# ReactiveBayes/RxInfer.jl

Hardware: NVIDIA H100
Metric: gaussian_messages_per_sec_batched_lgssm_d4_T1000 (higher is better)
Workload: dtype f32

## Files before the change

rxinfer.jl_b200/csrc/rxg_gain.cuh:

```cuda
#pragma once
#include <cooperative_groups.h>

#include "rxg_lgssm_common.cuh"

namespace rxg {
namespace cg = cooperative_groups;

constexpr int GS_CTAS = 8;
constexpr int GS_THREADS = 128;
constexpr int GS_NT = GS_CTAS * GS_THREADS;

struct ScanWs {
    double* fel;
    double* ftot;
    double* bel;
    double* btot;
};

template <int R, int C>
__device__ __forceinline__ Mat<double, R, C> ldcg_d(const double* p) {
    Mat<double, R, C> o;
#pragma unroll
    for (int i = 0; i < R * C; ++i) o.a[i] = __ldcg(p + i);
    return o;
}
template <int R, int C>
__device__ __forceinline__ Mat<double, R, C> ld_soa_d(const double* p, size_t n, size_t i) {
    Mat<double, R, C> o;
#pragma unroll
    for (int c = 0; c < R * C; ++c) o.a[c] = __ldcg(p + (size_t)c * n + i);
    return o;
}
template <int R, int C>
__device__ __forceinline__ void st_soa_d(double* p, size_t n, size_t i, const Mat<double, R, C>& A) {
#pragma unroll
    for (int c = 0; c < R * C; ++c) p[(size_t)c * n + i] = A.a[c];
}

template <int N, int K>
__device__ __forceinline__ Mat<double, N, K> solve_general(Mat<double, N, N> Mx, Mat<double, N, K> Rh) {
#pragma unroll
    for (int c = 0; c < N; ++c) {
        int p = c;
        double best = fabs(Mx(c, c));
#pragma unroll
        for (int r = c + 1; r < N; ++r) {
            const double v = fabs(Mx(r, c));
            if (v > best) { best = v; p = r; }
        }
#pragma unroll
        for (int r = c + 1; r < N; ++r) {
            if (r == p) {
#pragma unroll
                for (int j = c; j < N; ++j) { const double t = Mx(c, j); Mx(c, j) = Mx(r, j); Mx(r, j) = t; }
#pragma unroll
                for (int j = 0; j < K; ++j) { const double t = Rh(c, j); Rh(c, j) = Rh(r, j); Rh(r, j) = t; }
            }
        }
        const double inv = 1.0 / Mx(c, c);
#pragma unroll
        for (int r = c + 1; r < N; ++r) {
            const double f = Mx(r, c) * inv;
#pragma unroll
            for (int j = c + 1; j < N; ++j) Mx(r, j) = fma(-f, Mx(c, j), Mx(r, j));
#pragma unroll
            for (int j = 0; j < K; ++j) Rh(r, j) = fma(-f, Rh(c, j), Rh(r, j));
        }
    }
    Mat<double, N, K> X;
#pragma unroll
// ... 46 lines not shown
    Mat<double, D, D> Mx = mul(ei.C, ej.J);
#pragma unroll
    for (int i = 0; i < D; ++i) Mx(i, i) += 1.0;
    Mat<double, D, 2 * D> Rh;
#pragma unroll
    for (int i = 0; i < D; ++i)
#pragma unroll
        for (int j = 0; j < D; ++j) { Rh(i, j) = ei.A(i, j); Rh(i, D + j) = ei.C(i, j); }
    Mat<double, D, 2 * D> X = solve_general<D, 2 * D>(Mx, Rh);
    Mat<double, D, D> X1, X2;
#pragma unroll
    for (int i = 0; i < D; ++i)
#pragma unroll
        for (int j = 0; j < D; ++j) { X1(i, j) = X(i, j); X2(i, j) = X(i, D + j); }
    FwdEl<D> o;
    Mat<double, D, D> T2 = mul(ej.A, X2);
    o.C = sym_mul_nt_add(T2, ej.A, ej.C);
    if (!C_ONLY) {
        o.A = mul(ej.A, X1);
        Mat<double, D, D> JX = mul(ej.J, X1);
        Mat<double, D, D> AtJX = mul_tn(ei.A, JX);
#pragma unroll
        for (int i = 0; i < D; ++i)
#pragma unroll
            for (int j = 0; j <= i; ++j) {
                const double s = 0.5 * (AtJX(i, j) + AtJX(j, i)) + ei.J(i, j);
                o.J(i, j) = s; o.J(j, i) = s;
            }
    }
    return o;
}

template <int D>
__device__ __forceinline__ void bwd_store(double* p, size_t n, size_t i, const BwdEl<D>& e) {
    st_soa_d<D, D>(p, n, i, e.E);
    st_soa_d<D, D>(p + (size_t)D * D * n, n, i, e.L);
}
template <int D>
__device__ __forceinline__ BwdEl<D> bwd_load(const double* p, size_t n, size_t i) {
    BwdEl<D> e;
    e.E = ld_soa_d<D, D>(p, n, i);
    e.L = ld_soa_d<D, D>(p + (size_t)D * D * n, n, i);
    return e;
}
template <int D, bool L_ONLY>
__device__ __forceinline__ BwdEl<D> bwd_combine(const BwdEl<D>& early, const BwdEl<D>& late) {
    BwdEl<D> o;
    Mat<double, D, D> EL = mul(early.E, late.L);
    o.L = sym_mul_nt_add(EL, early.E, early.L);
    if (!L_ONLY) o.E = mul(early.E, late.E);
    return o;
}

template <int D, int M>
__global__ void __cluster_dims__(GS_CTAS, 1, 1) __launch_bounds__(GS_THREADS, 1)
gain_scan_kernel(const __grid_constant__ ModelF<D, M> mdl, GainWs ws, ScanWs sw, int T, int transition_first,
                 float* __restrict__ cov_shared_out, int* __restrict__ bad_out, const uint8_t* __restrict__ tmask,
                 const float* __restrict__ useq) {
    using TB = Tab<D, M>;
    cg::cluster_group cluster = cg::this_cluster();
    const int g = (int)cluster.block_rank() * GS_THREADS + (int)threadIdx.x;
    const int E = (T + GS_NT - 1) / GS_NT;
    const int k0 = g * E, k1 = min(k0 + E, T);
    constexpr int FE = 3 * D * D, BE = 2 * D * D;
    bool bad = false;

    const Mat<double, D, D> A = load_const<double, D, D>(mdl.A), P = load_const<double, D, D>(mdl.P);
    const Mat<double, M, D> B = load_const<double, M, D>(mdl.B);
    const Mat<double, M, M> Q = load_const<double, M, M>(mdl.Q);

    {
        FwdEl<D> acc = fwd_identity<D>();
        if (k0 < k1) {
            FwdEl<D> gen;
            {
                Mat<double, M, D> BP = mul(B, P);
                Mat<double, M, M> Sinn = sym_mul_nt_add(BP, B, Q);
                Chol<double, M> ch = cholesky<double, M, false>(Sinn, bad);
                Mat<double, D, M> V = solve_right_Lt(transpose(BP), ch.L);
                Mat<double, D, M> K = solve_right_L(V, ch.L);
                Mat<double, D, D> IKB = identity<double, D>();
#pragma unroll
                for (int i = 0; i < D; ++i)
#pragma unroll
                    for (int j = 0; j < D; ++j)
#pragma unroll
                        for (int k = 0; k < M; ++k) IKB(i, j) -= K(i, k) * B(k, j);
                gen.A = mul(IKB, A);
                gen.C = sym_downdate(P, V);
                Mat<double, M, D> BA = mul(B, A);
                Mat<double, M, D> Wm;
#pragma unroll
                for (int c = 0; c < D; ++c) {
                    Vec<double, M> col;
#pragma unroll
                    for (int r = 0; r < M; ++r) col(r) = BA(r, c);
                    Vec<double, M> z = solve_L(ch.L, col);
#pragma unroll
                    for (int r = 0; r < M; ++r) Wm(r, c) = z(r);
                }
                Mat<double, D, D> Z;
#pragma unroll
                for (int i = 0; i < D * D; ++i) Z.a[i] = 0.0;
                gen.J = sym_mul_nt_add(transpose(Wm), transpose(Wm), Z);
            }
            for (int k = k0; k < k1; ++k) {
                if (k == 0) {
                    Mat<double, D, D> S = load_const<double, D, D>(mdl.S0);
                    if (transition_first) { Mat<double, D, D> AS = mul(A, S); S = sym_mul_nt_add(AS, A, P); }
                    FwdEl<D> first;
#pragma unroll
                    for (int i = 0; i < D * D; ++i) { first.A.a[i] = 0.0; first.J.a[i] = 0.0; }
                    if (!tmask || tmask[0] != 0) {
                        Mat<double, M, D> BS = mul(B, S);
                        Mat<double, M, M> Sinn = sym_mul_nt_add(BS, B, Q);
                        Chol<double, M> ch = cholesky<double, M, false>(Sinn, bad);
                        Mat<double, D, M> V = solve_right_Lt(transpose(BS), ch.L);
                        first.C = sym_downdate(S, V);
                    } else {
                        first.C = S;
                    }
                    acc = first;
                } else {
                    const bool obs_k = !tmask || tmask[k] != 0;
                    if (obs_k) {
                        acc = (k == k0) ? gen : fwd_combine<D, false>(acc, gen);
                    } else {
                        FwdEl<D> miss;
                        miss.A = A; miss.C = P;
#pragma unroll
                        for (int i = 0; i < D * D; ++i) miss.J.a[i] = 0.0;
                        acc = (k == k0) ? miss : fwd_combine<D, false>(acc, miss);
                    }
                }
                if (E > 1) fwd_store<D>(sw.fel, T, k, acc);
            }
        }
        fwd_store<D>(sw.ftot, GS_NT, g, acc);
    }
    cluster.sync();
    int cur = 0;
    for (int off = 1; off < GS_NT; off <<= 1) {
        const double* src = sw.ftot + (size_t)cur * GS_NT * FE;
        double* dst = sw.ftot + (size_t)(cur ^ 1) * GS_NT * FE;
        FwdEl<D> mine = fwd_load<D>(src, GS_NT, g);
        if (g >= off && (g - off) * E < T && k0 < T) {
            FwdEl<D> prev = fwd_load<D>(src, GS_NT, g - off);
            mine = fwd_combine<D, false>(prev, mine);
        }
        fwd_store<D>(dst, GS_NT, g, mine);
        cluster.sync();
        cur ^= 1;
    }
    {
        const double* tot = sw.ftot + (size_t)cur * GS_NT * FE;
        if (E == 1) {
            if (g < T) store_d(ws.Sf + (size_t)g * D * D, ld_soa_d<D, D>(tot + (size_t)D * D * GS_NT, GS_NT, g));
        } else if (k0 < k1) {
            if (g == 0) {
                for (int k = k0; k < k1; ++k)
                    store_d(ws.Sf + (size_t)k * D * D, ld_soa_d<D, D>(sw.fel + (size_t)D * D * T, T, k));
            } else {
                const FwdEl<D> excl = fwd_load<D>(tot, GS_NT, g - 1);
                for (int k = k0; k < k1; ++k) {
                    const FwdEl<D> pk = fwd_load<D>(sw.fel, T, k);
                    store_d(ws.Sf + (size_t)k * D * D, fwd_combine<D, true>(excl, pk).C);
                }
            }
        }
    }
    cluster.sync();
    for (int t = g; t < T; t += GS_NT) {
        const Mat<double, D, D> Sf = ldcg_d<D, D>(ws.Sf + (size_t)t * D * D);
        Mat<double, D, D> Sp;
        if (t > 0) {
            Mat<double, D, D> Sfm = ldcg_d<D, D>(ws.Sf + (size_t)(t - 1) * D * D);
            Mat<double, D, D> AS = mul(A, Sfm);
            Sp = sym_mul_nt_add(AS, A, P);
        } else {
            Sp = load_const<double, D, D>(mdl.S0);
            if (transition_first) { Mat<double, D, D> AS = mul(A, Sp); Sp = sym_mul_nt_add(AS, A, P); }
        }
        const bool obs_t = !tmask || tmask[t] != 0;
        {
            Mat<double, D, M> K;
            Mat<double, M, M> Li;
            double cconst = 0.0;
#pragma unroll
            for (int i = 0; i < D * M; ++i) K.a[i] = 0.0;
#pragma unroll
            for (int i = 0; i < M * M; ++i) Li.a[i] = 0.0;
            if (obs_t) {
                Mat<double, M, D> BS = mul(B, Sp);
                Mat<double, M, M> Sinn = sym_mul_nt_add(BS, B, Q);
                Chol<double, M> ch = cholesky<double, M, true>(Sinn, bad);
                Mat<double, D, M> V = solve_right_Lt(transpose(BS), ch.L);
                K = solve_right_L(V, ch.L);
#pragma unroll
                for (int j = 0; j < M; ++j) {
                    Li(j, j) = ch.L(j, j);
#pragma unroll
                    for (int i = j + 1; i < M; ++i) {
                        double sacc = 0.0;
#pragma unroll
                        for (int k = j; k < i; ++k) sacc -= ch.L(i, k) * Li(k, j);
                        Li(i, j) = sacc * ch.L(i, i);
                    }
                }
                cconst = M * RXG_HALF_LOG_2PI - ch.neg_half_logdet;
            }
            Mat<double, D, D> IKB = identity<double, D>();
#pragma unroll
            for (int i = 0; i < D; ++i)
#pragma unroll
                for (int j = 0; j < D; ++j)
#pragma unroll
                    for (int k = 0; k < M; ++k) IKB(i, j) -= K(i, k) * B(k, j);
            Mat<double, D, D> F = (t > 0 || transition_first) ? mul(IKB, A) : IKB;
            float* rec = ws.fwd + (size_t)t * TB::FWD_REC;
            store_f(rec + TB::F_OFF, F);
            store_f(rec + TB::K_OFF, K);
            store_f(rec + TB::LI_OFF, Li);
            rec[TB::C_OFF] = (float)cconst;
            Vec<double, D> uu, gf;
#pragma unroll
            for (int i = 0; i < D; ++i) uu(i) = (double)(useq ? useq[(size_t)t * D + i] : mdl.u[i]);
            gf = mulv(IKB, uu);
            if (!(t > 0 || transition_first)) {
#pragma unroll
                for (int i = 0; i < D; ++i) gf(i) = 0.0;
            }
            store_fv(rec + TB::GF_OFF, gf);
            store_f(ws.sf + (size_t)t * TB::SF_REC, Sf);
        }
        float* brec = ws.bwd + (size_t)t * TB::BWD_REC;
        BwdEl<D> be;
        Vec<double, D> gb;
#pragma unroll
        for (int i = 0; i < D; ++i) gb(i) = 0.0;
        if (t < T - 1) {
            Mat<double, D, D> AS = mul(A, Sf);
            Mat<double, D, D> Sp1 = sym_mul_nt_add(AS, A, P);
            Chol<double, D> ch = cholesky<double, D, false>(Sp1, bad);
            Mat<double, D, D> U = solve_right_Lt(transpose(AS), ch.L);
            be.E = solve_right_L(U, ch.L);
            be.L = sym_downdate(Sf, U);
            Mat<double, D, D> Em = identity<double, D>();
            Mat<double, D, D> GA = mul(be.E, A);
#pragma unroll
            for (int i = 0; i < D * D; ++i) Em.a[i] -= GA.a[i];
            store_f(brec + TB::E_OFF, Em);
            store_f(brec + TB::G_OFF, be.E);
            Vec<double, D> uu;
#pragma unroll
            for (int i = 0; i < D; ++i) uu(i) = -(double)(useq ? useq[(size_t)(t + 1) * D + i] : mdl.u[i]);
            gb = mulv(be.E, uu);
        } else {
#pragma unroll
            for (int i = 0; i < D * D; ++i) be.E.a[i] = 0.0;
            be.L = Sf;
            store_f(brec + TB::E_OFF, identity<double, D>());
            store_f(brec + TB::G_OFF, be.E);
        }
        store_fv(brec + TB::GB_OFF, gb);
        bwd_store<D>(sw.bel, T, t, be);
    }
    cluster.sync();
    {
        BwdEl<D> acc;
        acc.E = identity<double, D>();
#pragma unroll
        for (int i = 0; i < D * D; ++i) acc.L.a[i] = 0.0;
        for (int r = k0; r < k1; ++r) {
            const int t = T - 1 - r;
            const BwdEl<D> el = bwd_load<D>(sw.bel, T, t);
            acc = (r == k0) ? el : bwd_combine<D, false>(el, acc);
            if (E > 1) bwd_store<D>(sw.bel, T, t, acc);
        }
        bwd_store<D>(sw.btot, GS_NT, g, acc);
    }
    cluster.sync();
    cur = 0;
    for (int off = 1; off < GS_NT; off <<= 1) {
        const double* src = sw.btot + (size_t)cur * GS_NT * BE;
        double* dst = sw.btot + (size_t)(cur ^ 1) * GS_NT * BE;
        BwdEl<D> mine = bwd_load<D>(src, GS_NT, g);
        if (g >= off && k0 < T) {
            BwdEl<D> prev = bwd_load<D>(src, GS_NT, g - off);
            mine = bwd_combine<D, false>(mine, prev);
        }
        bwd_store<D>(dst, GS_NT, g, mine);
        cluster.sync();
        cur ^= 1;
    }
    {
        const double* tot = sw.btot + (size_t)cur * GS_NT * BE;
        BwdEl<D> excl;
        if (E > 1 && g > 0 && k0 < k1) excl = bwd_load<D>(tot, GS_NT, g - 1);
        for (int r = k0; r < k1; ++r) {
            const int t = T - 1 - r;
            Mat<double, D, D> Ss;
            if (E == 1) {
                Ss = ld_soa_d<D, D>(tot + (size_t)D * D * GS_NT, GS_NT, g);
            } else {
                const BwdEl<D> pr = bwd_load<D>(sw.bel, T, t);
                Ss = (g == 0) ? pr.L : bwd_combine<D, true>(pr, excl).L;
            }
            store_f(ws.bwd + (size_t)t * TB::BWD_REC + TB::SS_OFF, Ss);
            if (cov_shared_out) store_f(cov_shared_out + (size_t)t * D * D, Ss);
        }
    }
    if (bad) atomicOr(bad_out, 1);
}

}
```

rxinfer.jl_b200/csrc/rxg_internal.h:

```cpp
#pragma once
#include <cuda_runtime.h>
#include <stdint.h>
#include <string.h>
#include <string>

#include "../../include/rxgauss.h"

struct rxg_ctx {
    int device = 0;
    cudaStream_t stream = nullptr;
    bool own_stream = false;
    std::string err;
    void* ws = nullptr;
    size_t ws_bytes = 0;
    void* stage = nullptr;
    size_t stage_bytes = 0;
    long long launches = 0;
    int sm_count = 132;
    bool gh_ready = false;
    bool gh_learn_ready = false;
    bool profile = false;
    cudaEvent_t ev[4] = {nullptr, nullptr, nullptr, nullptr};
    cudaStream_t s_in = nullptr, s_out = nullptr;
    cudaEvent_t ev_in[2] = {nullptr, nullptr}, ev_comp[2] = {nullptr, nullptr}, ev_out[2] = {nullptr, nullptr};
    cudaEvent_t ev_start = nullptr;
    void* h_tab = nullptr;
    size_t h_tab_bytes = 0;
    cudaEvent_t ev_tab = nullptr;
    cudaStream_t s_aux = nullptr;
    cudaEvent_t ev_aux[2] = {nullptr, nullptr};
    void* nccl_dl = nullptr;
    void* comm = nullptr;
    int nranks = 1, rank = 0;
    long long opt[RXG_OPT_COUNT_] = {};
    int* d_bad = nullptr;
    int* h_bad = nullptr;
    bool bad_pending = false;
    int peer_n = 0, peer_rank = 0;
    int* peer_flags[RXG_MAX_PEERS] = {};
    unsigned peer_epoch = 0;
    void* d_tmask = nullptr;
    size_t tmask_bytes = 0;
    void* d_useq = nullptr;
    size_t useq_bytes = 0;
    void* aux_buf[4] = {nullptr, nullptr, nullptr, nullptr};
    size_t aux_bytes[4] = {0, 0, 0, 0};
    void* fill_pool = nullptr;
    void* pred_buf = nullptr;
    size_t pred_bytes = 0;
};

namespace rxg {

int fail(rxg_ctx* ctx, int code, const char* fmt, ...);
int check_cuda(rxg_ctx* ctx, cudaError_t e, const char* what);
void* workspace(rxg_ctx* ctx, size_t bytes);
bool host_spd_inv(const float* a, int n, double* inv, double* logdet);
bool stochastic_columns(const float* p, int rows, int K);
bool positive(const float* p, int n);
void* staging(rxg_ctx* ctx, size_t bytes);
void gauss_hermite_31(double* t, double* w);
void* predict_scratch(rxg_ctx* ctx, size_t bytes);
int* bad_flag(rxg_ctx* ctx);
int begin_bad_flag(rxg_ctx* ctx);
int end_bad_flag(rxg_ctx* ctx, bool sync_now);

#define RXG_CUDA(ctx, call)                                         \
    do {                                                            \
        int _rc = ::rxg::check_cuda((ctx), (call), #call);          \
        if (_rc != RXG_OK) return _rc;                              \
    } while (0)

struct PeerOut {
    float* mean[RXG_MAX_PEERS - 1];
    float* cov[RXG_MAX_PEERS - 1];
    int n_mean;
    int n_cov;
};

struct LgssmCall {
    int d, m, T;
    int64_t batch;
    const float *A, *B, *P, *Q, *m0, *S0;
    const float* u;
    const float* useq = nullptr;
    const float* useq_host = nullptr;
    bool useq_chain = false;
    const float* mean0_chain = nullptr;
    const float* y;
    const uint8_t* ymask;
    const uint8_t* tmask = nullptr;
    int n_observed = -1;
    float* mean;
    float* cov;
    float* nle;
    int32_t* status;
    unsigned flags;
    bool smooth;
    bool tables_only = false;
    PeerOut po = {};
    bool want_cov_table = false;
    float* cov_table = nullptr;
// ... 41 lines not shown
```

rxinfer.jl_b200/csrc/rxg_lgssm.cu:

```cuda
#include <math.h>
#include <stdlib.h>

#include <utility>

#include "rxg_chain_step.cuh"
#include "rxg_gain.cuh"
#include "rxg_internal.h"
#include "rxg_linalg.cuh"
#include "rxg_lgssm_cluster.cuh"
#include "rxg_lgssm_common.cuh"
#include "rxg_lgssm_shared.cuh"
#include "rxg_lgssm_seg.cuh"
#include "rxg_sweep_select.h"

namespace rxg {

template <int D, int M, bool PER_CHAIN, bool SMOOTH, bool USEQ = false>
__global__ void __launch_bounds__(128)
lgssm_chain_kernel(const __grid_constant__ ModelF<D, M> mdl, PerChainPtrs pc,
                   const float* __restrict__ y, const uint8_t* __restrict__ mask,
                   float* __restrict__ mean, float* __restrict__ cov, float* __restrict__ nle,
                   int32_t* __restrict__ status, int T, int64_t batch, int transition_first,
                   const float* __restrict__ useq = nullptr, int64_t ustride = 0, int uchain = 0) {
    const int64_t b = (int64_t)blockIdx.x * blockDim.x + threadIdx.x;
    if (b >= batch) return;

    Mat<float, D, D> A, P, S0;
    Mat<float, M, D> B;
    Mat<float, M, M> Q;
    Vec<float, D> mu, u;
    if (PER_CHAIN) {
        A = load_strided<float, D, D>(pc.A + b, batch);
        B = load_strided<float, M, D>(pc.B + b, batch);
        P = load_strided<float, D, D>(pc.P + b, batch);
        Q = load_strided<float, M, M>(pc.Q + b, batch);
        S0 = load_strided<float, D, D>(pc.S0 + b, batch);
#pragma unroll
        for (int i = 0; i < D; ++i) mu(i) = __ldg(pc.m0 + i * batch + b);
#pragma unroll
        for (int i = 0; i < D; ++i) u(i) = pc.u ? __ldg(pc.u + i * batch + b) : 0.f;
    } else {
        A = load_const<float, D, D>(mdl.A);
        B = load_const<float, M, D>(mdl.B);
        P = load_const<float, D, D>(mdl.P);
        Q = load_const<float, M, M>(mdl.Q);
        S0 = load_const<float, D, D>(mdl.S0);
#pragma unroll
        for (int i = 0; i < D; ++i) { mu(i) = mdl.m0[i]; u(i) = mdl.u[i]; }
    }
    Mat<float, D, D> S = S0;
    bool bad = false;
    double acc_nle = 0.0;
    const bool want_nle = (nle != nullptr);

    float ynext[M];
// ... 301 lines not shown
                         int write_cov, std::integer_sequence<int, I...>) {
    return (launch_sweep_if<D, M, I>(pick, ctx, c, mdl, ws, write_cov) || ...);
}

template <int D, int M>
static int launch_shared(rxg_ctx* ctx, LgssmCall& c, const ModelF<D, M>& mdl, const GainWs& ws, int write_cov,
                         const SweepPick& p) {
    const int pick = sweep_pick_index(p);
    if (ctx->profile) cudaEventRecord(ctx->ev[1], ctx->stream);
    if (!launch_sweep<D, M>(pick, ctx, c, mdl, ws, write_cov, std::make_integer_sequence<int, SWEEP_PICK_COUNT>{}))
        return fail(ctx, RXG_ERR_UNSUPPORTED, "lgssm: no lgssm_shared_kernel instantiation for sweep pick %d", pick);
    if (ctx->profile) cudaEventRecord(ctx->ev[2], ctx->stream);
    ctx->launches += 1;
    c.fused_peer_stores = p.peer;
    return check_cuda(ctx, cudaGetLastError(), "lgssm_shared_kernel launch");
}

template <int D, int M>
static bool seg_sweep_eligible(const LgssmCall& c) {
    using ST = SegTab<D, M>;
    if (!c.smooth || c.nle || D * D > 16) return false;
    const int nseg = (c.T + ST::L - 1) / ST::L;
    const size_t smem = (size_t)nseg * 2 * D * 32 * 4 + (size_t)8 * 2 * ST::L * ST::REC * 4;
    return smem <= 200 * 1024;
}
template <int D, int M>
static int launch_seg(rxg_ctx* ctx, LgssmCall& c, const ModelF<D, M>& mdl, const GainWs& ws, const SegWs& sw, int write_cov,
                      bool hints) {
    using ST = SegTab<D, M>;
    constexpr int NW = 8;
    const int nseg = (c.T + ST::L - 1) / ST::L;
    seg_tables_kernel<D, M><<<(nseg + 63) / 64, 64, 0, ctx->stream>>>(ws, sw, c.T);
    const size_t smem = (size_t)nseg * 2 * D * 32 * 4 + (size_t)NW * 2 * ST::L * ST::REC * 4;
    const int64_t ntiles = (c.batch + 31) / 32;
    const unsigned grid = (unsigned)(ntiles < ctx->sm_count ? ntiles : ctx->sm_count);
    bool has_u = false;
    for (int i = 0; i < D; ++i) has_u |= (mdl.u[i] != 0.f);
#define RXG_LAUNCH_SEG(OF, HI)                                                                                        \
    do {                                                                                                               \
        RXG_CUDA(ctx, cudaFuncSetAttribute(lgssm_seg_kernel<D, M, NW, OF, HI>, cudaFuncAttributeMaxDynamicSharedMemorySize, (int)smem)); \
        if (ctx->profile) cudaEventRecord(ctx->ev[1], ctx->stream);                                                    \
        lgssm_seg_kernel<D, M, NW, OF, HI><<<grid, 32 * NW, smem, ctx->stream>>>(mdl, sw, c.y, c.mean, c.cov, c.T, c.batch, \
                                                                                 write_cov, c.mean0_chain, c.po, nseg);  \
    } while (0)
    (void)hints;
    if (has_u) RXG_LAUNCH_SEG(true, 1); else RXG_LAUNCH_SEG(false, 1);
#undef RXG_LAUNCH_SEG
    if (ctx->profile) cudaEventRecord(ctx->ev[2], ctx->stream);
    ctx->launches += 2;
    c.fused_peer_stores = false;
    return check_cuda(ctx, cudaGetLastError(), "lgssm_seg_kernel launch");
}

template <int D, int M>
static int launch_cluster_if_eligible(rxg_ctx* ctx, LgssmCall& c, const ModelF<D, M>& mdl, const GainWs& ws, float* cl_tab,
                                      int write_cov, bool& launched) {
    launched = false;
    if constexpr (D * D <= 16 && M >= D) {
        using CT = ClusterTab<D, M>;
        bool offset = false;
        for (int i = 0; i < D; ++i) offset |= (mdl.u[i] != 0.f);
        const bool aligned = (((uintptr_t)c.y | (uintptr_t)c.mean | (uintptr_t)c.cov) & 15) == 0;
        if (!c.smooth || c.nle || c.useq || offset || c.mean0_chain || c.batch % 32 != 0 || !aligned ||
            ctx->opt[RXG_OPT_SWEEP_VARIANT] != 0 || ctx->opt[RXG_OPT_FORCE_CPT] != 0)
            return RXG_OK;
        const size_t smem = CT::smem_bytes(c.T);
        int smem_max = 0;
        RXG_CUDA(ctx, cudaDeviceGetAttribute(&smem_max, cudaDevAttrMaxSharedMemoryPerBlockOptin, ctx->device));
        if (smem > (size_t)smem_max) return RXG_OK;
        const bool peer = c.po.n_mean > 0 || c.po.n_cov > 0;
        auto kern = peer ? lgssm_cluster_sweep_kernel<D, M, true> : lgssm_cluster_sweep_kernel<D, M, false>;
        RXG_CUDA(ctx, cudaFuncSetAttribute(kern, cudaFuncAttributeMaxDynamicSharedMemorySize, (int)smem));
        cudaLaunchConfig_t cfg = {};
        cudaLaunchAttribute attr[1];
        attr[0].id = cudaLaunchAttributeClusterDimension;
        attr[0].val.clusterDim.x = CL_CTAS;
        attr[0].val.clusterDim.y = 1;
        attr[0].val.clusterDim.z = 1;
        cfg.gridDim = dim3((unsigned)(c.batch / 32 * CL_CTAS));
        cfg.blockDim = dim3(32 * CL_WARPS);
        cfg.dynamicSmemBytes = smem;
        cfg.stream = ctx->stream;
        cfg.attrs = attr;
        cfg.numAttrs = 1;
        int nclusters = 0;
        RXG_CUDA(ctx, cudaOccupancyMaxActiveClusters(&nclusters, kern, &cfg));
        if (nclusters < 1) return RXG_OK;

        const int spc = CT::spc(c.T);
        cluster_tables_kernel<D, M><<<1, 256, 0, ctx->stream>>>(ws, cl_tab, c.T, spc);
        if (ctx->profile) cudaEventRecord(ctx->ev[1], ctx->stream);
        RXG_CUDA(ctx, cudaLaunchKernelEx(&cfg, kern, (const float*)ws.fwd, (const float*)ws.bwd, (const float*)cl_tab, c.y,
                                         c.mean, c.cov, c.T, c.batch, write_cov, mdl, c.po));
        if (ctx->profile) cudaEventRecord(ctx->ev[2], ctx->stream);
        ctx->launches += 2;
        c.fused_peer_stores = peer;
        launched = true;
        return check_cuda(ctx, cudaGetLastError(), "lgssm_cluster_sweep_kernel launch");
    }
    return RXG_OK;
}

template <int D, int M>
static int run_shared_family(rxg_ctx* ctx, LgssmCall& c) {
    using TB = Tab<D, M>;
    ModelF<D, M> mdl = {};
    fill_model<D, M>(mdl, c);
    const size_t T = (size_t)c.T;
    size_t off = 0;
    auto carve = [&](size_t bytes) { size_t o = off; off += (bytes + 255) / 256 * 256; return o; };
    const size_t o_fwd = carve(T * TB::FWD_REC * sizeof(float));
    const size_t o_bwd = carve(T * TB::BWD_REC * sizeof(float));
    const size_t o_sf = carve(T * TB::SF_REC * sizeof(float));
    const size_t o_Sp = carve(T * D * D * sizeof(double));
    const size_t o_Sf = carve(T * D * D * sizeof(double));
    const size_t o_Cc = carve(T * D * D * sizeof(double));
    const size_t o_Gd = carve(T * D * D * sizeof(double));
    const size_t o_fel = carve(T * 3 * D * D * sizeof(double));
    const size_t o_ftot = carve((size_t)2 * GS_NT * 3 * D * D * sizeof(double));
    const size_t o_bel = carve(T * 2 * D * D * sizeof(double));
    const size_t o_btot = carve((size_t)2 * GS_NT * 2 * D * D * sizeof(double));
    using ST = SegTab<D, M>;
    const size_t nseg = (T + ST::L - 1) / ST::L;
    const size_t o_srec_t = carve(T * ST::REC * sizeof(float)), o_snrec = carve(T * ST::NREC * sizeof(float));
    const size_t o_ssrec = carve(nseg * ST::SREC * sizeof(float));
    const size_t o_ctab = carve(c.want_cov_table ? T * D * D * sizeof(float) : 0);
    const size_t o_cl = carve(ClusterTab<D, M>::table_floats(c.T) * sizeof(float));
    char* base = (char*)workspace(ctx, off);
    if (!base) return RXG_ERR_CUDA;
    GainWs ws;
    ws.fwd = (float*)(base + o_fwd); ws.bwd = (float*)(base + o_bwd); ws.sf = (float*)(base + o_sf);
    ws.Sp = (double*)(base + o_Sp); ws.Sf = (double*)(base + o_Sf);
    ws.Cc = (double*)(base + o_Cc); ws.Gd = (double*)(base + o_Gd);
    ScanWs sw;
    sw.fel = (double*)(base + o_fel); sw.ftot = (double*)(base + o_ftot);
    sw.bel = (double*)(base + o_bel); sw.btot = (double*)(base + o_btot);

    const int tf = (c.flags & RXG_TRANSITION_FIRST) ? 1 : 0;
    const bool cov_shared = (c.flags & RXG_COV_SHARED_OUT) != 0;
    c.cov_table = (c.want_cov_table && c.smooth) ? (float*)(base + o_ctab) : nullptr;
    if (ctx->profile) cudaEventRecord(ctx->ev[0], ctx->stream);
    float* cov_once = (cov_shared && c.cov && c.smooth) ? c.cov : (c.smooth ? c.cov_table : nullptr);
    const float* useq_tab = c.useq_chain ? nullptr : c.useq;
    if (ctx->opt[RXG_OPT_GAIN_SEQ] != 0) {
        gain_riccati_seq<D, M><<<1, 32, 0, ctx->stream>>>(mdl, ws, c.T, tf, bad_flag(ctx), c.tmask);
        gain_tables<D, M><<<(c.T + 63) / 64, 64, 0, ctx->stream>>>(mdl, ws, c.T, tf, bad_flag(ctx), c.tmask, useq_tab);
        ctx->launches += 2;
        if (c.smooth) {
            gain_smooth_seq<D, M><<<1, 32, 0, ctx->stream>>>(ws, c.T, cov_once);
            ctx->launches += 1;
        }
    } else {
        gain_scan_kernel<D, M><<<GS_CTAS, GS_THREADS, 0, ctx->stream>>>(mdl, ws, sw, c.T, tf, cov_once, bad_flag(ctx), c.tmask,
                                                                          useq_tab);
        ctx->launches += 1;
    }
    if (!c.smooth && cov_shared && c.cov) {
        const int n = c.T * D * D;
        copy_table_kernel<<<(n + 255) / 256, 256, 0, ctx->stream>>>(ws.sf, TB::SF_REC, D * D, c.T, c.cov);
        ctx->launches += 1;
    }
    int rc = check_cuda(ctx, cudaGetLastError(), "gain table kernels launch");
    if (rc != RXG_OK) return rc;
    if (c.ev_tables) RXG_CUDA(ctx, cudaEventRecord(c.ev_tables, ctx->stream));
    if (c.tables_only) return RXG_OK;
    const int write_cov = (c.cov != nullptr && !cov_shared) ? 1 : 0;
    bool launched = false;
    rc = launch_cluster_if_eligible<D, M>(ctx, c, mdl, ws, (float*)(base + o_cl), write_cov, launched);
    if (rc != RXG_OK || launched) return rc;
    const long long variant = ctx->opt[RXG_OPT_SWEEP_VARIANT];
    if (variant == 3 && !c.useq && seg_sweep_eligible<D, M>(c)) {
        SegWs sgw;
        sgw.rec = (float*)(base + o_srec_t); sgw.nrec = (float*)(base + o_snrec); sgw.srec = (float*)(base + o_ssrec);
        return launch_seg<D, M>(ctx, c, mdl, ws, sgw, write_cov, variant == 3);
    }
    SweepQuery q = {};
    q.d = D;
    q.m = M;
    q.batch = c.batch;
    q.sm_count = ctx->sm_count;
    q.force_cpt = ctx->opt[RXG_OPT_FORCE_CPT];
    q.aligned16 = (((uintptr_t)c.y | (uintptr_t)c.mean | (uintptr_t)c.cov | (uintptr_t)c.nle | (uintptr_t)c.mean0_chain |
                    (uintptr_t)(c.useq_chain ? c.useq : nullptr)) & 15) == 0;
    q.smooth = c.smooth;
    q.evid = c.nle != nullptr;
    for (int i = 0; i < D; ++i) q.offset |= (mdl.u[i] != 0.f);
    q.input = !c.useq ? InputSeq::none : (c.useq_chain ? InputSeq::per_chain : InputSeq::shared);
    q.peer_out = c.po.n_mean > 0 || c.po.n_cov > 0;
    q.sweep_variant = variant;
    return launch_shared<D, M>(ctx, c, mdl, ws, write_cov, select_shared_sweep(q));
}

template <int D, int M>
int run_dm(rxg_ctx* ctx, LgssmCall& c) {
    const bool per_chain = (c.flags & (RXG_MODEL_PER_CHAIN | RXG_PATH_PER_CHAIN)) != 0 || c.ymask != nullptr;
    if (per_chain) return run_chain_family<D, M>(ctx, c);
    int rc = run_shared_family<D, M>(ctx, c);
    if (rc == RXG_OK && c.status) rc = fill_status_from_flag(ctx, c.status, c.batch);
    return rc;
}

#ifdef RXG_INST_D
template int run_dm<RXG_INST_D, RXG_INST_M>(rxg_ctx*, LgssmCall&);
#else
extern template int run_dm<1, 1>(rxg_ctx*, LgssmCall&);
extern template int run_dm<2, 1>(rxg_ctx*, LgssmCall&);
extern template int run_dm<2, 2>(rxg_ctx*, LgssmCall&);
// ... 36 lines not shown
```

rxinfer.jl_b200/csrc/rxg_lgssm_cluster.cuh:

```cuda
#pragma once
#include <cooperative_groups.h>

#include "rxg_lgssm_common.cuh"
#include "rxg_lgssm_shared.cuh"

namespace rxg {

constexpr int CL_CTAS = 8;
constexpr int CL_WARPS = 8;
constexpr int CL_L = 16;

template <int D, int M>
struct ClusterTab {
    static constexpr int FK = pad4(D * D) + pad4(D * M);
    static constexpr int EG = 2 * pad4(D * D);
    static constexpr int REC = 2 * pad4(D * D);
    static constexpr int PSI_OFF = pad4(D * D);
    static_assert(Tab<D, M>::F_OFF == 0 && Tab<D, M>::K_OFF == pad4(D * D) && Tab<D, M>::E_OFF == 0 &&
                      Tab<D, M>::G_OFF == pad4(D * D),
                  "the staged prefixes are the first FK / EG floats of the gain records");

    static __host__ __device__ int spc(int T) { return ((T + CL_L - 1) / CL_L + CL_CTAS - 1) / CL_CTAS; }
    static size_t table_floats(int T) { return (size_t)(CL_CTAS * spc(T) + CL_CTAS) * REC; }
    static size_t smem_bytes(int T) {
        const size_t S = (size_t)spc(T) * CL_L;
        return 4 * (S * (M * 32 + FK + EG) + (size_t)(spc(T) + CL_CTAS) * REC + (size_t)spc(T) * D * 32 + 2 * D * 32);
    }
};

template <int D, int M>
__global__ void __launch_bounds__(256) cluster_tables_kernel(GainWs ws, float* __restrict__ tab, int T, int spc) {
    using TB = Tab<D, M>;
    using CT = ClusterTab<D, M>;
    const int nsub = CL_CTAS * spc;
    for (int j = threadIdx.x; j < nsub; j += blockDim.x) {
        const int a = j * CL_L, e = min(a + CL_L, T);
        Mat<double, D, D> Phi = identity<double, D>(), Psi = identity<double, D>();
        for (int t = a; t < e; ++t) {
            Phi = mul(load_const<double, D, D>(ws.fwd + (size_t)t * TB::FWD_REC + TB::F_OFF), Phi);
            Psi = mul(Psi, load_const<double, D, D>(ws.bwd + (size_t)t * TB::BWD_REC + TB::G_OFF));
        }
        store_f(tab + (size_t)j * CT::REC, Phi);
        store_f(tab + (size_t)j * CT::REC + CT::PSI_OFF, Psi);
    }
    __syncthreads();
    for (int r = threadIdx.x; r < CL_CTAS; r += blockDim.x) {
        Mat<double, D, D> Phi = identity<double, D>(), Psi = identity<double, D>();
        for (int j = r * spc; j < (r + 1) * spc; ++j) {
            Phi = mul(load_const<double, D, D>(tab + (size_t)j * CT::REC), Phi);
            Psi = mul(Psi, load_const<double, D, D>(tab + (size_t)j * CT::REC + CT::PSI_OFF));
        }
        store_f(tab + (size_t)(nsub + r) * CT::REC, Phi);
        store_f(tab + (size_t)(nsub + r) * CT::REC + CT::PSI_OFF, Psi);
    }
}

template <int D>
__device__ __forceinline__ void affine_step(const float* Mx, float (&v)[D], const float (&w)[D]) {
    float Mr[pad4(D * D)];
    load_smem<pad4(D * D)>(Mx, Mr);
    float n[D];
#pragma unroll
    for (int i = 0; i < D; ++i) {
        float a = w[i];
#pragma unroll
        for (int j = 0; j < D; ++j) a = __fmaf_rn(Mr[i * D + j], v[j], a);
        n[i] = a;
    }
#pragma unroll
    for (int i = 0; i < D; ++i) v[i] = n[i];
}

template <int D, int M>
__device__ __forceinline__ void store_cov_span(const float* __restrict__ bwd_tab, float* __restrict__ cov, int64_t batch,
                                               int T) {
    using TB = Tab<D, M>;
    constexpr int NT = 32 * CL_WARPS;
    const int n4 = (int)(batch / 4);
    const int span = D * D * T;
    const int64_t base = (int64_t)blockIdx.x * span;
    float4* out = reinterpret_cast<float4*>(cov) + base;
    const int step_rows = NT / n4, step_cols = NT % n4;
    int i = (int)threadIdx.x;
    const int64_t q = base + i;
    int row = (int)(q / n4), col = (int)(q - (int64_t)row * n4);
    int cur = -1;
    float4 v = {};
    for (; i < span; i += NT) {
        if (row != cur) {
            cur = row;
            const float s = bwd_tab[(size_t)(row / (D * D)) * TB::BWD_REC + TB::SS_OFF + row % (D * D)];
            v = make_float4(s, s, s, s);
        }
        __stcs(out + i, v);
        row += step_rows;
        col += step_cols;
        if (col >= n4) { col -= n4; ++row; }
    }
}

template <int D, int M, bool PEER>
__global__ void __launch_bounds__(32 * CL_WARPS, 2)
lgssm_cluster_sweep_kernel(const float* __restrict__ fwd_tab, const float* __restrict__ bwd_tab,
                           const float* __restrict__ cl_tab, const float* __restrict__ y, float* __restrict__ mean,
                           float* __restrict__ cov, int T, int64_t batch, int write_cov,
                           const __grid_constant__ ModelF<D, M> mdl, const __grid_constant__ PeerOut po) {
// ... 248 lines not shown
```

Measured before the change: 150.0 billion.

## Move gain-scan combine into shared/DSMEM, tree-reduce cluster tables, cache host queries

The forward and backward cross-thread scans in the gain kernel now run through shared memory, with an intra-CTA Hillis-Steele pass followed by a DSMEM exchange of CTA totals. This replaces global-memory ping-pong buffers that needed a cluster.sync per round. The cluster tables kernel now uses 8 blocks that reduce products with a parallel tree in shared memory, instead of one block doing serial per-thread products. Host-side occupancy, device-attribute and smem-attribute queries are cached, and missing-observation elements are built with branch-free selects. The scan adds more dynamic shared memory and needs careful barrier ordering.

```diff
diff --git a/rxinfer.jl_b200/csrc/rxg_gain.cuh b/rxinfer.jl_b200/csrc/rxg_gain.cuh
--- a/rxinfer.jl_b200/csrc/rxg_gain.cuh
+++ b/rxinfer.jl_b200/csrc/rxg_gain.cuh
@@ -12,10 +12,13 @@
 
 struct ScanWs {
     double* fel;
-    double* ftot;
     double* bel;
-    double* btot;
 };
+
+constexpr int GS_SLOTS = GS_THREADS + GS_CTAS;
+
+template <int D>
+constexpr size_t gain_scan_smem_bytes() { return (size_t)GS_SLOTS * 3 * D * D * sizeof(double); }
 
 template <int R, int C>
 __device__ __forceinline__ Mat<double, R, C> ldcg_d(const double* p) {
@@ -168,25 +171,104 @@
     return o;
 }
 
+template <int R, int C>
+__device__ __forceinline__ Mat<double, R, C> ld_soa_sh(const double* p, int n, int i) {
+    Mat<double, R, C> o;
+#pragma unroll
+    for (int c = 0; c < R * C; ++c) o.a[c] = p[c * n + i];
+    return o;
+}
+template <int D>
+__device__ __forceinline__ void el_load(const double* p, int n, int i, FwdEl<D>& e) {
+    e.A = ld_soa_sh<D, D>(p, n, i);
+    e.C = ld_soa_sh<D, D>(p + D * D * n, n, i);
+    e.J = ld_soa_sh<D, D>(p + 2 * D * D * n, n, i);
+}
+template <int D>
+__device__ __forceinline__ void el_load(const double* p, int n, int i, BwdEl<D>& e) {
+    e.E = ld_soa_sh<D, D>(p, n, i);
+    e.L = ld_soa_sh<D, D>(p + D * D * n, n, i);
+}
+template <int D>
+__device__ __forceinline__ void el_store(double* p, int n, int i, const FwdEl<D>& e) { fwd_store<D>(p, n, i, e); }
+template <int D>
+__device__ __forceinline__ void el_store(double* p, int n, int i, const BwdEl<D>& e) { bwd_store<D>(p, n, i, e); }
+
+template <int D>
+__device__ __forceinline__ FwdEl<D> scan_op(const FwdEl<D>& pre, const FwdEl<D>& x) { return fwd_combine<D, false>(pre, x); }
+template <int D>
+__device__ __forceinline__ BwdEl<D> scan_op(const BwdEl<D>& pre, const BwdEl<D>& x) { return bwd_combine<D, false>(x, pre); }
+
+template <class El>
+__device__ __forceinline__ El cluster_scan(cg::cluster_group& cluster, const El& own, bool active, double* sm, int T,
+                                           int E) {
+    constexpr int CTA_ROUNDS = 7, ROUNDS = 11;
+    const int tid = (int)threadIdx.x, rank = (int)cluster.block_rank();
+    el_store(sm, GS_SLOTS, tid, own);
+    __syncthreads();
+#pragma unroll 1
+    for (int round = 0; round < ROUNDS; ++round) {
+        if (round == CTA_ROUNDS) {
+            cluster.sync();
+            if (tid < GS_CTAS) {
+                El t;
+                el_load(cluster.map_shared_rank(sm, tid), GS_SLOTS, GS_THREADS - 1, t);
+                el_store(sm, GS_SLOTS, GS_THREADS + tid, t);
+            }
+            asm volatile("barrier.cluster.arrive.release.aligned;\n" ::: "memory");
+            __syncthreads();
+        }
+        if (round == ROUNDS - 1) asm volatile("barrier.cluster.wait.acquire.aligned;\n" ::: "memory");
+        bool take;
+        int pi, mi;
+        if (round < CTA_ROUNDS) {
+            const int off = 1 << round;
+            take = active && tid >= off;
+            pi = tid - off; mi = tid;
+        } else if (round < ROUNDS - 1) {
+            const int off = 1 << (round - CTA_ROUNDS);
+            take = tid < GS_CTAS && tid >= off && tid * GS_THREADS * E < T;
+            pi = GS_THREADS + tid - off; mi = GS_THREADS + tid;
+        } else {
+            take = active && rank > 0;
+            pi = GS_THREADS + rank - 1; mi = tid;
+        }
+        El mine;
+        if (take) {
+            El prev;
+            el_load(sm, GS_SLOTS, pi, prev);
+            el_load(sm, GS_SLOTS, mi, mine);
+            mine = scan_op(prev, mine);
+        }
+        __syncthreads();
+        if (take) el_store(sm, GS_SLOTS, mi, mine);
+        __syncthreads();
+    }
+    El mine;
+    el_load(sm, GS_SLOTS, tid, mine);
+    return mine;
+}
+
 template <int D, int M>
 __global__ void __cluster_dims__(GS_CTAS, 1, 1) __launch_bounds__(GS_THREADS, 1)
 gain_scan_kernel(const __grid_constant__ ModelF<D, M> mdl, GainWs ws, ScanWs sw, int T, int transition_first,
                  float* __restrict__ cov_shared_out, int* __restrict__ bad_out, const uint8_t* __restrict__ tmask,
                  const float* __restrict__ useq) {
     using TB = Tab<D, M>;
+    extern __shared__ double sm[];
     cg::cluster_group cluster = cg::this_cluster();
-    const int g = (int)cluster.block_rank() * GS_THREADS + (int)threadIdx.x;
+    const int rank = (int)cluster.block_rank(), tid = (int)threadIdx.x;
+    const int g = rank * GS_THREADS + tid;
     const int E = (T + GS_NT - 1) / GS_NT;
     const int k0 = g * E, k1 = min(k0 + E, T);
-    constexpr int FE = 3 * D * D, BE = 2 * D * D;
     bool bad = false;
 
     const Mat<double, D, D> A = load_const<double, D, D>(mdl.A), P = load_const<double, D, D>(mdl.P);
     const Mat<double, M, D> B = load_const<double, M, D>(mdl.B);
     const Mat<double, M, M> Q = load_const<double, M, M>(mdl.Q);
 
+    FwdEl<D> acc = fwd_identity<D>();
     {
-        FwdEl<D> acc = fwd_identity<D>();
         if (k0 < k1) {
             FwdEl<D> gen;
             {
@@ -238,51 +320,31 @@
                     }
                     acc = first;
                 } else {
-                    const bool obs_k = !tmask || tmask[k] != 0;
-                    if (obs_k) {
-                        acc = (k == k0) ? gen : fwd_combine<D, false>(acc, gen);
-                    } else {
-                        FwdEl<D> miss;
-                        miss.A = A; miss.C = P;
-#pragma unroll
-                        for (int i = 0; i < D * D; ++i) miss.J.a[i] = 0.0;
-                        acc = (k == k0) ? miss : fwd_combine<D, false>(acc, miss);
+                    const bool miss = tmask && tmask[k] == 0;
+                    FwdEl<D> el;
+#pragma unroll
+                    for (int i = 0; i < D * D; ++i) {
+                        el.A.a[i] = miss ? A.a[i] : gen.A.a[i];
+                        el.C.a[i] = miss ? P.a[i] : gen.C.a[i];
+                        el.J.a[i] = miss ? 0.0 : gen.J.a[i];
                     }
+                    acc = (k == k0) ? el : fwd_combine<D, false>(acc, el);
                 }
                 if (E > 1) fwd_store<D>(sw.fel, T, k, acc);
             }
         }
-        fwd_store<D>(sw.ftot, GS_NT, g, acc);
-    }
-    cluster.sync();
-    int cur = 0;
-    for (int off = 1; off < GS_NT; off <<= 1) {
-        const double* src = sw.ftot + (size_t)cur * GS_NT * FE;
-        double* dst = sw.ftot + (size_t)(cur ^ 1) * GS_NT * FE;
-        FwdEl<D> mine = fwd_load<D>(src, GS_NT, g);
-        if (g >= off && (g - off) * E < T && k0 < T) {
-            FwdEl<D> prev = fwd_load<D>(src, GS_NT, g - off);
-            mine = fwd_combine<D, false>(prev, mine);
-        }
-        fwd_store<D>(dst, GS_NT, g, mine);
-        cluster.sync();
-        cur ^= 1;
-    }
+    }
+    acc = cluster_scan(cluster, acc, k0 < T, sm, T, E);
     {
-        const double* tot = sw.ftot + (size_t)cur * GS_NT * FE;
         if (E == 1) {
-            if (g < T) store_d(ws.Sf + (size_t)g * D * D, ld_soa_d<D, D>(tot + (size_t)D * D * GS_NT, GS_NT, g));
+            if (g < T) store_d(ws.Sf + (size_t)g * D * D, acc.C);
         } else if (k0 < k1) {
-            if (g == 0) {
-                for (int k = k0; k < k1; ++k)
-                    store_d(ws.Sf + (size_t)k * D * D, ld_soa_d<D, D>(sw.fel + (size_t)D * D * T, T, k));
-            } else {
-                const FwdEl<D> excl = fwd_load<D>(tot, GS_NT, g - 1);
-                for (int k = k0; k < k1; ++k) {
-                    const FwdEl<D> pk = fwd_load<D>(sw.fel, T, k);
-                    store_d(ws.Sf + (size_t)k * D * D, fwd_combine<D, true>(excl, pk).C);
-                }
-            }
+            if (g > 0) {
+                el_load(sm, GS_SLOTS, tid > 0 ? tid - 1 : GS_THREADS + rank - 1, acc);
+            }
+            for (int k = k0; k < k1; ++k)
+                store_d(ws.Sf + (size_t)k * D * D, g == 0 ? ld_soa_d<D, D>(sw.fel + (size_t)D * D * T, T, k)
+                                                          : fwd_combine<D, true>(acc, fwd_load<D>(sw.fel, T, k)).C);
         }
     }
     cluster.sync();
@@ -382,45 +444,29 @@
         bwd_store<D>(sw.bel, T, t, be);
     }
     cluster.sync();
+    BwdEl<D> bacc;
+    bacc.E = identity<double, D>();
+#pragma unroll
+    for (int i = 0; i < D * D; ++i) bacc.L.a[i] = 0.0;
+    for (int r = k0; r < k1; ++r) {
+        const int t = T - 1 - r;
+        const BwdEl<D> el = bwd_load<D>(sw.bel, T, t);
+        bacc = (r == k0) ? el : bwd_combine<D, false>(el, bacc);
+        if (E > 1) bwd_store<D>(sw.bel, T, t, bacc);
+    }
+    bacc = cluster_scan(cluster, bacc, k0 < T, sm, T, E);
     {
-        BwdEl<D> acc;
-        acc.E = identity<double, D>();
-#pragma unroll
-        for (int i = 0; i < D * D; ++i) acc.L.a[i] = 0.0;
-        for (int r = k0; r < k1; ++r) {
-            const int t = T - 1 - r;
-            const BwdEl<D> el = bwd_load<D>(sw.bel, T, t);
-            acc = (r == k0) ? el : bwd_combine<D, false>(el, acc);
-            if (E > 1) bwd_store<D>(sw.bel, T, t, acc);
-        }
-        bwd_store<D>(sw.btot, GS_NT, g, acc);
-    }
-    cluster.sync();
-    cur = 0;
-    for (int off = 1; off < GS_NT; off <<= 1) {
-        const double* src = sw.btot + (size_t)cur * GS_NT * BE;
-        double* dst = sw.btot + (size_t)(cur ^ 1) * GS_NT * BE;
-        BwdEl<D> mine = bwd_load<D>(src, GS_NT, g);
-        if (g >= off && k0 < T) {
-            BwdEl<D> prev = bwd_load<D>(src, GS_NT, g - off);
-            mine = bwd_combine<D, false>(mine, prev);
-        }
-        bwd_store<D>(dst, GS_NT, g, mine);
-        cluster.sync();
-        cur ^= 1;
-    }
-    {
-        const double* tot = sw.btot + (size_t)cur * GS_NT * BE;
-        BwdEl<D> excl;
-        if (E > 1 && g > 0 && k0 < k1) excl = bwd_load<D>(tot, GS_NT, g - 1);
+        if (E > 1 && g > 0) {
+            el_load(sm, GS_SLOTS, tid > 0 ? tid - 1 : GS_THREADS + rank - 1, bacc);
+        }
         for (int r = k0; r < k1; ++r) {
             const int t = T - 1 - r;
             Mat<double, D, D> Ss;
             if (E == 1) {
-                Ss = ld_soa_d<D, D>(tot + (size_t)D * D * GS_NT, GS_NT, g);
+                Ss = bacc.L;
             } else {
                 const BwdEl<D> pr = bwd_load<D>(sw.bel, T, t);
-                Ss = (g == 0) ? pr.L : bwd_combine<D, true>(pr, excl).L;
+                Ss = (g == 0) ? pr.L : bwd_combine<D, true>(pr, bacc).L;
             }
             store_f(ws.bwd + (size_t)t * TB::BWD_REC + TB::SS_OFF, Ss);
             if (cov_shared_out) store_f(cov_shared_out + (size_t)t * D * D, Ss);
diff --git a/rxinfer.jl_b200/csrc/rxg_internal.h b/rxinfer.jl_b200/csrc/rxg_internal.h
--- a/rxinfer.jl_b200/csrc/rxg_internal.h
+++ b/rxinfer.jl_b200/csrc/rxg_internal.h
@@ -2,7 +2,9 @@
 #include <cuda_runtime.h>
 #include <stdint.h>
 #include <string.h>
+#include <map>
 #include <string>
+#include <utility>
 
 #include "../../include/rxgauss.h"
 
@@ -48,6 +50,8 @@
     void* fill_pool = nullptr;
     void* pred_buf = nullptr;
     size_t pred_bytes = 0;
+    int smem_optin = -1;
+    std::map<std::pair<const void*, size_t>, int> max_clusters;
 };
 
 namespace rxg {
diff --git a/rxinfer.jl_b200/csrc/rxg_lgssm.cu b/rxinfer.jl_b200/csrc/rxg_lgssm.cu
--- a/rxinfer.jl_b200/csrc/rxg_lgssm.cu
+++ b/rxinfer.jl_b200/csrc/rxg_lgssm.cu
@@ -1,6 +1,8 @@
 #include <math.h>
 #include <stdlib.h>
 
+#include <map>
+#include <mutex>
 #include <utility>
 
 #include "rxg_chain_step.cuh"
@@ -408,6 +410,17 @@
     return check_cuda(ctx, cudaGetLastError(), "lgssm_seg_kernel launch");
 }
 
+static int allow_dyn_smem(rxg_ctx* ctx, const void* kern, size_t bytes) {
+    static std::mutex mu;
+    static std::map<std::pair<int, const void*>, size_t> allowed;
+    std::lock_guard<std::mutex> lock(mu);
+    size_t& cur = allowed[{ctx->device, kern}];
+    if (cur >= bytes) return RXG_OK;
+    RXG_CUDA(ctx, cudaFuncSetAttribute(kern, cudaFuncAttributeMaxDynamicSharedMemorySize, (int)bytes));
+    cur = bytes;
+    return RXG_OK;
+}
+
 template <int D, int M>
 static int launch_cluster_if_eligible(rxg_ctx* ctx, LgssmCall& c, const ModelF<D, M>& mdl, const GainWs& ws, float* cl_tab,
                                       int write_cov, bool& launched) {
@@ -421,12 +434,13 @@
             ctx->opt[RXG_OPT_SWEEP_VARIANT] != 0 || ctx->opt[RXG_OPT_FORCE_CPT] != 0)
             return RXG_OK;
         const size_t smem = CT::smem_bytes(c.T);
-        int smem_max = 0;
-        RXG_CUDA(ctx, cudaDeviceGetAttribute(&smem_max, cudaDevAttrMaxSharedMemoryPerBlockOptin, ctx->device));
-        if (smem > (size_t)smem_max) return RXG_OK;
+        if (ctx->smem_optin < 0)
+            RXG_CUDA(ctx, cudaDeviceGetAttribute(&ctx->smem_optin, cudaDevAttrMaxSharedMemoryPerBlockOptin, ctx->device));
+        if (smem > (size_t)ctx->smem_optin) return RXG_OK;
         const bool peer = c.po.n_mean > 0 || c.po.n_cov > 0;
         auto kern = peer ? lgssm_cluster_sweep_kernel<D, M, true> : lgssm_cluster_sweep_kernel<D, M, false>;
-        RXG_CUDA(ctx, cudaFuncSetAttribute(kern, cudaFuncAttributeMaxDynamicSharedMemorySize, (int)smem));
+        int rc = allow_dyn_smem(ctx, (const void*)kern, smem);
+        if (rc != RXG_OK) return rc;
         cudaLaunchConfig_t cfg = {};
         cudaLaunchAttribute attr[1];
         attr[0].id = cudaLaunchAttributeClusterDimension;
@@ -439,12 +453,20 @@
         cfg.stream = ctx->stream;
         cfg.attrs = attr;
         cfg.numAttrs = 1;
-        int nclusters = 0;
-        RXG_CUDA(ctx, cudaOccupancyMaxActiveClusters(&nclusters, kern, &cfg));
-        if (nclusters < 1) return RXG_OK;
+        const auto occ_key = std::make_pair((const void*)kern, smem);
+        auto occ = ctx->max_clusters.find(occ_key);
+        if (occ == ctx->max_clusters.end()) {
+            int nclusters = 0;
+            RXG_CUDA(ctx, cudaOccupancyMaxActiveClusters(&nclusters, kern, &cfg));
+            occ = ctx->max_clusters.emplace(occ_key, nclusters).first;
+        }
+        if (occ->second < 1) return RXG_OK;
 
         const int spc = CT::spc(c.T);
-        cluster_tables_kernel<D, M><<<1, 256, 0, ctx->stream>>>(ws, cl_tab, c.T, spc);
+        const size_t tab_smem = CT::tables_smem_bytes(c.T);
+        rc = allow_dyn_smem(ctx, (const void*)cluster_tables_kernel<D, M>, tab_smem);
+        if (rc != RXG_OK) return rc;
+        cluster_tables_kernel<D, M><<<CL_CTAS, CL_TAB_THREADS, tab_smem, ctx->stream>>>(ws, cl_tab, c.T, spc);
         if (ctx->profile) cudaEventRecord(ctx->ev[1], ctx->stream);
         RXG_CUDA(ctx, cudaLaunchKernelEx(&cfg, kern, (const float*)ws.fwd, (const float*)ws.bwd, (const float*)cl_tab, c.y,
                                          c.mean, c.cov, c.T, c.batch, write_cov, mdl, c.po));
@@ -473,9 +495,7 @@
     const size_t o_Cc = carve(T * D * D * sizeof(double));
     const size_t o_Gd = carve(T * D * D * sizeof(double));
     const size_t o_fel = carve(T * 3 * D * D * sizeof(double));
-    const size_t o_ftot = carve((size_t)2 * GS_NT * 3 * D * D * sizeof(double));
     const size_t o_bel = carve(T * 2 * D * D * sizeof(double));
-    const size_t o_btot = carve((size_t)2 * GS_NT * 2 * D * D * sizeof(double));
     using ST = SegTab<D, M>;
     const size_t nseg = (T + ST::L - 1) / ST::L;
     const size_t o_srec_t = carve(T * ST::REC * sizeof(float)), o_snrec = carve(T * ST::NREC * sizeof(float));
@@ -489,8 +509,8 @@
     ws.Sp = (double*)(base + o_Sp); ws.Sf = (double*)(base + o_Sf);
     ws.Cc = (double*)(base + o_Cc); ws.Gd = (double*)(base + o_Gd);
     ScanWs sw;
-    sw.fel = (double*)(base + o_fel); sw.ftot = (double*)(base + o_ftot);
-    sw.bel = (double*)(base + o_bel); sw.btot = (double*)(base + o_btot);
+    sw.fel = (double*)(base + o_fel);
+    sw.bel = (double*)(base + o_bel);
 
     const int tf = (c.flags & RXG_TRANSITION_FIRST) ? 1 : 0;
     const bool cov_shared = (c.flags & RXG_COV_SHARED_OUT) != 0;
@@ -507,8 +527,11 @@
             ctx->launches += 1;
         }
     } else {
-        gain_scan_kernel<D, M><<<GS_CTAS, GS_THREADS, 0, ctx->stream>>>(mdl, ws, sw, c.T, tf, cov_once, bad_flag(ctx), c.tmask,
-                                                                          useq_tab);
+        constexpr size_t gs_smem = gain_scan_smem_bytes<D>();
+        const int rc_smem = allow_dyn_smem(ctx, (const void*)gain_scan_kernel<D, M>, gs_smem);
+        if (rc_smem != RXG_OK) return rc_smem;
+        gain_scan_kernel<D, M><<<GS_CTAS, GS_THREADS, gs_smem, ctx->stream>>>(mdl, ws, sw, c.T, tf, cov_once, bad_flag(ctx),
+                                                                                c.tmask, useq_tab);
         ctx->launches += 1;
     }
     if (!c.smooth && cov_shared && c.cov) {
diff --git a/rxinfer.jl_b200/csrc/rxg_lgssm_cluster.cuh b/rxinfer.jl_b200/csrc/rxg_lgssm_cluster.cuh
--- a/rxinfer.jl_b200/csrc/rxg_lgssm_cluster.cuh
+++ b/rxinfer.jl_b200/csrc/rxg_lgssm_cluster.cuh
@@ -22,36 +22,78 @@
 
     static __host__ __device__ int spc(int T) { return ((T + CL_L - 1) / CL_L + CL_CTAS - 1) / CL_CTAS; }
     static size_t table_floats(int T) { return (size_t)(CL_CTAS * spc(T) + CL_CTAS) * REC; }
+    static size_t tables_smem_bytes(int T) { return (size_t)2 * D * D * spc(T) * (CL_L / 2) * sizeof(double); }
     static size_t smem_bytes(int T) {
         const size_t S = (size_t)spc(T) * CL_L;
         return 4 * (S * (M * 32 + FK + EG) + (size_t)(spc(T) + CL_CTAS) * REC + (size_t)spc(T) * D * 32 + 2 * D * 32);
     }
 };
 
+constexpr int CL_TAB_THREADS = 256;
+
+template <int D>
+__device__ __forceinline__ Mat<double, D, D> ld_node(const double* p, int n, int i) {
+    Mat<double, D, D> o;
+#pragma unroll
+    for (int c = 0; c < D * D; ++c) o.a[c] = p[c * n + i];
+    return o;
+}
+template <int D>
+__device__ __forceinline__ void st_node(double* p, int n, int i, const Mat<double, D, D>& A) {
+#pragma unroll
+    for (int c = 0; c < D * D; ++c) p[c * n + i] = A.a[c];
+}
+
 template <int D, int M>
-__global__ void __launch_bounds__(256) cluster_tables_kernel(GainWs ws, float* __restrict__ tab, int T, int spc) {
+__global__ void __launch_bounds__(CL_TAB_THREADS) cluster_tables_kernel(GainWs ws, float* __restrict__ tab, int T, int spc) {
     using TB = Tab<D, M>;
     using CT = ClusterTab<D, M>;
-    const int nsub = CL_CTAS * spc;
-    for (int j = threadIdx.x; j < nsub; j += blockDim.x) {
-        const int a = j * CL_L, e = min(a + CL_L, T);
-        Mat<double, D, D> Phi = identity<double, D>(), Psi = identity<double, D>();
-        for (int t = a; t < e; ++t) {
-            Phi = mul(load_const<double, D, D>(ws.fwd + (size_t)t * TB::FWD_REC + TB::F_OFF), Phi);
-            Psi = mul(Psi, load_const<double, D, D>(ws.bwd + (size_t)t * TB::BWD_REC + TB::G_OFF));
-        }
-        store_f(tab + (size_t)j * CT::REC, Phi);
-        store_f(tab + (size_t)j * CT::REC + CT::PSI_OFF, Psi);
-    }
-    __syncthreads();
-    for (int r = threadIdx.x; r < CL_CTAS; r += blockDim.x) {
-        Mat<double, D, D> Phi = identity<double, D>(), Psi = identity<double, D>();
-        for (int j = r * spc; j < (r + 1) * spc; ++j) {
-            Phi = mul(load_const<double, D, D>(tab + (size_t)j * CT::REC), Phi);
-            Psi = mul(Psi, load_const<double, D, D>(tab + (size_t)j * CT::REC + CT::PSI_OFF));
-        }
-        store_f(tab + (size_t)(nsub + r) * CT::REC, Phi);
-        store_f(tab + (size_t)(nsub + r) * CT::REC + CT::PSI_OFF, Psi);
+    constexpr int HL = CL_L / 2;
+    extern __shared__ double ct_smem[];
+    const int r = (int)blockIdx.x, nleaf = spc * HL, t_base = r * spc * CL_L;
+    double* const phi = ct_smem;
+    double* const psi = ct_smem + (size_t)D * D * nleaf;
+    for (int task = threadIdx.x; task < 2 * nleaf; task += CL_TAB_THREADS) {
+        const bool is_psi = task >= nleaf;
+        const int p = is_psi ? task - nleaf : task, t0 = t_base + 2 * p;
+        Mat<double, D, D> X[2];
+#pragma unroll
+        for (int s = 0; s < 2; ++s) {
+            const int t = t0 + s;
+            X[s] = t >= T ? identity<double, D>()
+                 : is_psi ? load_const<double, D, D>(ws.bwd + (size_t)t * TB::BWD_REC + TB::G_OFF)
+                          : load_const<double, D, D>(ws.fwd + (size_t)t * TB::FWD_REC + TB::F_OFF);
+        }
+        if (is_psi) st_node<D>(psi, nleaf, p, mul(X[0], X[1]));
+        else st_node<D>(phi, nleaf, p, mul(X[1], X[0]));
+    }
+    __syncthreads();
+    for (int w = 1; w < nleaf; w <<= 1) {
+        const int nodes = (nleaf + 2 * w - 1) / (2 * w);
+        for (int task = threadIdx.x; task < 2 * nodes; task += CL_TAB_THREADS) {
+            const bool is_psi = task >= nodes;
+            const int i = (is_psi ? task - nodes : task) * 2 * w;
+            if (i + w < nleaf) {
+                double* const b = is_psi ? psi : phi;
+                const Mat<double, D, D> lo = ld_node<D>(b, nleaf, i), hi = ld_node<D>(b, nleaf, i + w);
+                st_node<D>(b, nleaf, i, is_psi ? mul(lo, hi) : mul(hi, lo));
+            }
+        }
+        __syncthreads();
+        if (2 * w == HL) {
+            for (int task = threadIdx.x; task < 2 * spc; task += CL_TAB_THREADS) {
+                const bool is_psi = task >= spc;
+                const int jl = is_psi ? task - spc : task;
+                store_f(tab + (size_t)(r * spc + jl) * CT::REC + (is_psi ? CT::PSI_OFF : 0),
+                        ld_node<D>(is_psi ? psi : phi, nleaf, jl * HL));
+            }
+            __syncthreads();
+        }
+    }
+    if (threadIdx.x < 2) {
+        const bool is_psi = threadIdx.x == 1;
+        store_f(tab + (size_t)(CL_CTAS * spc + r) * CT::REC + (is_psi ? CT::PSI_OFF : 0),
+                ld_node<D>(is_psi ? psi : phi, nleaf, 0));
     }
 }
 
```

Measured after the change: 153.3 billion, median of 6. 2.2% higher.
